# DanielaCourel/smoothed_particle_hydrodynamics

Measured on AMD Instinct MI355X. Metric: Mparticle-steps/sec (whole node), dam-break, higher is better.
Workload: dtype f32

## Files before the change

smoothed_particle_hydrodynamics_amd/csrc/full_tiled.h:

```cpp
#pragma once

#include "launch_policy.h"
#include "common_kernels.h"
#include "full_kernels.h"
#include "neighbor_lists.h"
#include "slab_kernels.h"

#if defined(SPH_ABLATE) && !defined(SPH_DIAGNOSTIC_BUILD)
#error "SPH_ABLATE is for diagnostic builds only: add -DSPH_DIAGNOSTIC_BUILD (tools/build_variant.sh does)"
#endif

#ifdef SPH_TRIPCOUNT
#ifndef SPH_DIAGNOSTIC_BUILD
#error "SPH_TRIPCOUNT is for diagnostic builds only: add -DSPH_DIAGNOSTIC_BUILD"
#endif
enum {
   TRIP_D_WAVES = 0, TRIP_D_CHUNKS_W, TRIP_D_TEST8_W, TRIP_D_TEST8_L, TRIP_D_SLOTS_L, TRIP_D_POPS_W,
   TRIP_D_POPS_L, TRIP_D_POPLOOPS_W, TRIP_D_SUMTRIPS_W, TRIP_D_SUMSLOTS_W, TRIP_D_LISTED_L, TRIP_D_LANES_L,
   TRIP_A_WAVES = 16, TRIP_A_PTRIPS_W, TRIP_A_CNT_L, TRIP_A_VTRIPS_W, TRIP_A_NV_L, TRIP_A_LANES_L,
   TRIP_COUNT = 32
};
__device__ unsigned long long g_trip[TRIP_COUNT];
struct TripCounters {
   unsigned int v[16];
// ... 703 lines not shown
   return block < count ? b1 + xcd_workgroup(block, count) : -1;
}

template <bool UNIT_SCALE>
__device__ __forceinline__ void fused_integrate(const FusedStep& fs, const PairConsts& k,
                                                const CellGrid& g, int p, bool live, float4 x,
                                                float4 a, int wg_index)
{
   double ke = 0.0, pe = 0.0;
   uint32_t c = 0xffffffffu;
   float4 v = make_float4(0.f, 0.f, 0.f, 0.f);
   if (live) {
      v = fs.velp_in[p];
      integrate_particle<UNIT_SCALE>(k, x, v, a, ke, pe);
      fs.posm_out[p] = x;
      fs.velp_out[p] = v;
      int cx, cy, cz;
      c = cell_of(g, x.x, x.y, x.z, cx, cy, cz);
      fs.key[p] = c;
   }
   count_cell_runs(c, live, p, fs.cell_count, fs.slot, (uint32_t)g.ncells);
   if (fs.slab) {
      bool to_left = false, to_right = false;
      if (live) {
         const int ob = fs.meta[META_OWN_BEGIN], oe = fs.meta[META_OWN_END];
         const int lo_end = min(fs.meta[META_BND_LO_END], oe);
         const int hi_begin = min(max(fs.meta[META_BND_HI_BEGIN], lo_end), oe);
         const int plane = cell_coord(x.z, g.inv, g.nz_global);
         const bool near_left = fs.zone.have_left && plane < fs.zone.lo + fs.zone.halo;
         const bool near_right = fs.zone.have_right && plane >= fs.zone.hi - fs.zone.halo;
         if ((p >= ob && p < lo_end) || (p >= hi_begin && p < oe)) {
            to_left = near_left;
            to_right = near_right;
         } else if (near_left || near_right) {
            atomicOr(&fs.meta[META_ERRORS], 8);
         }
      }
      if (fs.zone.have_left) {
         const int s = msg_reserve(&fs.left->header[0], to_left);
         if (to_left) {
            if (s < fs.msg_capacity) {
               fs.left->rec[2 * s] = x;
               fs.left->rec[2 * s + 1] = v;
            } else {
               atomicOr(&fs.meta[META_ERRORS], 2);
            }
         }
      }
      if (fs.zone.have_right) {
         const int s = msg_reserve(&fs.right->header[0], to_right);
         if (to_right) {
            if (s < fs.msg_capacity) {
               fs.right->rec[2 * s] = x;
               fs.right->rec[2 * s + 1] = v;
            } else {
               atomicOr(&fs.meta[META_ERRORS], 2);
            }
         }
      }
   }
   __shared__ double s_ke[TILE_THREADS / SPH_WAVE], s_pe[TILE_THREADS / SPH_WAVE];
#pragma unroll
   for (int d = SPH_WAVE / 2; d > 0; d >>= 1) {
      ke += __shfl_down(ke, d);
      pe += __shfl_down(pe, d);
   }
   const int lane = threadIdx.x & (SPH_WAVE - 1), w = threadIdx.x / SPH_WAVE;
   if (lane == 0) {
      s_ke[w] = ke;
      s_pe[w] = pe;
   }
   __syncthreads();
   if (threadIdx.x == 0) {
      double sa = 0.0, sb = 0.0;
#pragma unroll
      for (int q = 0; q < TILE_THREADS / SPH_WAVE; q++) {
         sa += s_ke[q];
         sb += s_pe[q];
      }
      fs.epart[2 * wg_index + 0] = sa;
      fs.epart[2 * wg_index + 1] = sb;
   }
   __syncthreads();
}

template <bool UNIT_SCALE, bool UNIFORM_MASS, bool WIDE, bool FAST>
__device__ __forceinline__ float4
accel_from_lists(int p, int cnt, const ListReader& lr, const TileDesc& d,
                 const float4* __restrict__ posm, const float4* __restrict__ velB,
                 const float* __restrict__ rho, const float* __restrict__ auxc, const PairConsts& k)
{
   const float4 pi = posm[p];
   AccelState s;
   accel_begin(k, s, pi, velB[p], rho[p]);
   const bool in_range = accel_operands_in_range(k);
   int first_v = 0;
   if (FAST) first_v = visc_first(cnt, s.visc_scale);
   if constexpr (FAST) {
      const int lastb = cnt > 0 ? (cnt - 1) >> 3 : 0;
      uint4 blk = lr.block(0);
      for (int j0 = 0; j0 < cnt; j0 += 8) {
         uint32_t entry[8];
         list_block_entries(blk, entry);
         blk = lr.block(min((j0 >> 3) + 1, lastb));
         float4 pj[8];
         float cj[8];
#pragma unroll
         for (int u = 0; u < 8; u++) {
            const uint32_t e = j0 + u < cnt ? entry[u] : entry[0];
            const int q = ListEntry<WIDE>::tile(e) - ListEntry<WIDE>::shift(d, e);
            pj[u] = posm[q];
            cj[u] = auxc[q];
         }
#pragma unroll
         for (int u = 0; u < 8; u++) {
            if (j0 + u < cnt) {
               float dx, dy, dz;
               float dd = sqrt_rn(dist2(pi.x, pi.y, pi.z, pj[u].x, pj[u].y, pj[u].z, dx, dy, dz));
               if (!UNIT_SCALE) dd *= k.sim_scale;
               accel_pair_fast_pressure<UNIT_SCALE>(k, s, dx, dy, dz, dd, cj[u]);
            }
         }
      }
      for (int j0 = first_v; j0 < cnt; j0 += VISC_UNROLL) {
         float4 pj[VISC_UNROLL], vj[VISC_UNROLL];
#pragma unroll
         for (int u = 0; u < VISC_UNROLL; u++) {
            const uint32_t e = lr.entry((uint32_t)min(j0 + u, cnt - 1));
            const int q = ListEntry<WIDE>::tile(e) - ListEntry<WIDE>::shift(d, e);
            pj[u] = posm[q];
            vj[u] = velB[q];
         }
#pragma unroll
         for (int u = 0; u < VISC_UNROLL; u++) {
            if (j0 + u < cnt) {
               float dx, dy, dz;
               float dd = sqrt_rn(dist2(pi.x, pi.y, pi.z, pj[u].x, pj[u].y, pj[u].z, dx, dy, dz));
               if (!UNIT_SCALE) dd *= k.sim_scale;
               accel_pair_fast_viscous(k, s, dd, vj[u].x, vj[u].y, vj[u].z, vj[u].w);
            }
         }
      }
      accel_fast_finish(k, s);
      return accel_end<UNIT_SCALE>(k, s);
   }
   constexpr int U = 4;
   for (int j0 = 0; j0 < cnt; j0 += U) {
      float4 pj[U], vj[U];
      float cj[U];
#pragma unroll
      for (int u = 0; u < U; u++) {
         const int j = min(j0 + u, cnt - 1);
         const uint32_t e = lr.entry((uint32_t)j);
         const int q = ListEntry<WIDE>::tile(e) - ListEntry<WIDE>::shift(d, e);
         pj[u] = posm[q];
         cj[u] = auxc[q];
         vj[u] = make_float4(0.f, 0.f, 0.f, 0.f);
         if (!FAST || j >= first_v) vj[u] = velB[q];
      }
#pragma unroll
      for (int u = 0; u < U; u++) {
         if (j0 + u < cnt) {
            float dx, dy, dz;
            const float d2 = dist2(pi.x, pi.y, pi.z, pj[u].x, pj[u].y, pj[u].z, dx, dy, dz);
            float dd = sqrt_rn(d2);
            if (!UNIT_SCALE) dd *= k.sim_scale;
            if (FAST) {
               accel_pair_fast_pressure<UNIT_SCALE>(k, s, dx, dy, dz, dd, cj[u]);
               if (j0 + u >= first_v) accel_pair_fast_viscous(k, s, dd, vj[u].x, vj[u].y, vj[u].z, vj[u].w);
            } else {
               accel_pair<UNIT_SCALE>(k, s, dx, dy, dz, dd, UNIFORM_MASS ? pi.w : pj[u].w, vj[u].x, vj[u].y,
                                      vj[u].z, vj[u].w, cj[u], in_range);
            }
         }
      }
   }
   if (FAST) accel_fast_finish(k, s);
   return accel_end<UNIT_SCALE>(k, s);
}

template <bool UNIT_SCALE, bool UNIFORM_MASS, bool WIDE, bool FAST>
__global__ void __launch_bounds__(TILE_THREADS, ACCEL_BLOCKS)
k_full_accel_lists(const float4* __restrict__ posm, const float4* __restrict__ velB,
                   const float* __restrict__ rho, const float* __restrict__ auxc,
                   const int32_t* __restrict__ ncount, const uint32_t* __restrict__ cell_start,
                   const int32_t* __restrict__ meta, CellGrid g, PairConsts k,
                   float4* __restrict__ acc, const TileDesc* __restrict__ desc,
                   const uint32_t* __restrict__ nlist, const uint32_t* __restrict__ nlist_overflow,
                   int tile_cap, const int32_t* __restrict__ tile_stats,
                   const uint32_t* __restrict__ giveup, int part, int list_cap,
                   int* __restrict__ tile_feedback, FusedStep fs, int tile_cap_density)
{
   PHASE_BEGIN();
   __shared__ AccelLds L;
   float4* xyzc = reinterpret_cast<float4*>(tile_lds_dynamic);
   constexpr int BATCH = TILE_BATCH;

   const int begin = meta[META_SUM_BEGIN], end = meta[META_SUM_END];
   const int ob = meta[META_OWN_BEGIN], oe = meta[META_OWN_END];
   const int tid = threadIdx.x;
   const int wgs = tile_stats[TSTAT_BLOCKS];
   const int mapped = accel_part_workgroup(part, blockIdx.x, wgs, begin, meta);
   const int wg = mapped < 0 ? 0 : mapped;
   const int p0 = begin + wg * TILE_THREADS;
   if (blockIdx.x == 0 && tid == 0) {
      tile_feedback[TSTAT_NO_LIST] = tile_stats[TSTAT_NO_LIST];
      if (fs.slab && part == 1) {
         if (fs.left) fs.left->header[1] = fs.msg_capacity;
         if (fs.right) fs.right->header[1] = fs.msg_capacity;
      }
   }
   const bool own = mapped >= 0 && !(p0 >= end || p0 + TILE_THREADS <= ob || p0 >= oe) &&
                    accel_part_has(part, p0, meta);
   const uint32_t gave_up = own ? nlist_overflow[wg] : LISTS_NONE;
   int desc_word = 0;
   if (tid < (int)(sizeof(TileDesc) / sizeof(int))) desc_word = reinterpret_cast<const int*>(&desc[wg])[tid];
   if ((int)blockIdx.x < tile_stats[TSTAT_GIVEUP_ACCEL]) {
      const int g0 = begin + (int)giveup[blockIdx.x] * TILE_THREADS;
      const int gp = g0 + tid;
      const bool mine = gp < end && gp >= ob && gp < oe && accel_part_has(part, g0, meta);
      const int gwg = (int)giveup[blockIdx.x];
      const uint32_t glists = nlist_overflow[gwg];
      if (glists != LISTS_NONE) {
         tile_desc_load(desc, gwg, L.desc);
         if (mine) {
            const int gcnt = ncount[gp];
            const ListReader glr(nlist, gwg, list_cap, tid);
            if (glists == LISTS_SOME && gcnt > 0 && glr.no_list())
               accel_untiled<UNIT_SCALE, FAST>(gp, posm, velB, rho, auxc, cell_start, g, k, acc, ncount);
            else
               acc[gp] = accel_from_lists<UNIT_SCALE, UNIFORM_MASS, WIDE, FAST>(gp, gcnt, glr, L.desc, posm, velB,
                                                                                rho, auxc, k);
         }
         __syncthreads();
      } else if (mine) {
         accel_untiled<UNIT_SCALE, FAST>(gp, posm, velB, rho, auxc, cell_start, g, k, acc, ncount);
      }
      if (fs.on && accel_part_has(part, g0, meta)) {
         float4 gx = make_float4(0.f, 0.f, 0.f, 0.f), ga = gx;
         if (mine) {
            gx = posm[gp];
            ga = acc[gp];
         }
         fused_integrate<UNIT_SCALE>(fs, k, g, gp, mine, gx, ga, (int)giveup[blockIdx.x]);
      }
   }
   if (gave_up == LISTS_NONE) return;
   if (tid < (int)(sizeof(TileDesc) / sizeof(int))) reinterpret_cast<int*>(&L.desc)[tid] = desc_word;
   __syncthreads();
   PHASE_MARK(16);
   const int total = L.desc.total;
   if (total > tile_cap || total > tile_cap_density) return;
   int B[9], D[9];
#pragma unroll
   for (int kk = 0; kk < 9; kk++) {
      B[kk] = L.desc.B[kk];
      D[kk] = L.desc.D[kk];
   }
   float4 buf[BATCH];
   float cbuf[BATCH];
#if defined(SPH_ABLATE) && SPH_ABLATE == 23
#pragma unroll
   for (int r = 0; r < BATCH; r++) {
      buf[r] = make_float4(0.f, 0.f, 0.f, 0.f);
      cbuf[r] = 0.f;
   }
   const int filled = 0;
#else
#pragma unroll
   for (int r = 0; r < BATCH; r++) {
      const int idx = min(tid + r * TILE_THREADS, total - 1);
      int d = D[0];
#pragma unroll
      for (int kk = 1; kk < 9; kk++) d = (idx >= B[kk]) ? D[kk] : d;
      buf[r] = posm[idx - d];
      cbuf[r] = auxc[idx - d];
   }
   const int filled = total;
#endif

   const int col = tid;
   const int p = p0 + col;
   const bool live = p < end && p >= ob && p < oe;
   float4 pi = make_float4(0.f, 0.f, 0.f, 0.f);
   float4 vi = pi;
   float rho_i = 0.0f;
   int cnt = 0;
   if (live) {
      pi = posm[p];
      vi = velB[p];
      rho_i = rho[p];
      cnt = ncount[p];
   }

   const ListReader lr(nlist, wg, list_cap, col);
   uint32_t entry[LIST_BLOCK_ENTRIES];
   uint4 next_blk = lr.block(0);

#pragma unroll
   for (int r = 0; r < BATCH; r++) {
      const int idx = tid + r * TILE_THREADS;
      if (idx < filled) xyzc[idx] = make_float4(buf[r].x, buf[r].y, buf[r].z, cbuf[r]);
   }
   for (int base = BATCH * TILE_THREADS; base < filled; base += BATCH * TILE_THREADS) {
#pragma unroll
      for (int r = 0; r < BATCH; r++) {
         const int idx = min(base + tid + r * TILE_THREADS, filled - 1);
         int d = D[0];
#pragma unroll
         for (int kk = 1; kk < 9; kk++) d = (idx >= B[kk]) ? D[kk] : d;
         buf[r] = posm[idx - d];
         cbuf[r] = auxc[idx - d];
      }
#pragma unroll
      for (int r = 0; r < BATCH; r++) {
         const int idx = base + tid + r * TILE_THREADS;
         if (idx < filled) xyzc[idx] = make_float4(buf[r].x, buf[r].y, buf[r].z, cbuf[r]);
      }
   }
   __syncthreads();

   PHASE_MARK(17);
   AccelState s;
   accel_begin(k, s, pi, vi, rho_i);
   const bool in_range = accel_operands_in_range(k);
   bool no_list = false;
   if (gave_up == LISTS_SOME && cnt > 0) no_list = next_blk.x == NLIST_NO_LIST;
   int first_v = 0;
   if (FAST) first_v = visc_first(cnt, s.visc_scale);
   if (no_list) cnt = 0;
#if defined(SPH_ABLATE) && (SPH_ABLATE == 21 || SPH_ABLATE == 23)
   cnt = 0;
#endif
   const int lastb = cnt > 0 ? (cnt - 1) >> 3 : 0;
   if constexpr (FAST) {
      const int self_tile = live ? p + L.desc.D[4] : 0;
      const float4 self = xyzc[self_tile];
      const float self_c = (k.hscaled * k.hscaled) * (s.pi_div_rhoi2 * self.w) +
                           ((self.x - self.x) + (self.y - self.y) + (self.z - self.z));
      const bool odd_lane = __any(!__builtin_isfinite(s.pi_div_rhoi2) || !__builtin_isfinite(self_c));
      TRIP(TripCounters trips; trips.wave(TRIP_A_WAVES - 16, true); trips.lane(TRIP_A_CNT_L - 16, (unsigned)cnt);
           trips.lane(TRIP_A_LANES_L - 16, live ? 1u : 0u); trips.lane(TRIP_A_NV_L - 16, (unsigned)(cnt - first_v));)
      for (int j0 = 0; __any(j0 < cnt); j0 += LIST_BLOCK_ENTRIES) {
         TRIP(trips.wave(TRIP_A_PTRIPS_W - 16, true);)
         list_block_entries(next_blk, entry);
         next_blk = lr.block(min((j0 >> 3) + 1, lastb));
         float dx[LIST_BLOCK_ENTRIES], dy[LIST_BLOCK_ENTRIES], dz[LIST_BLOCK_ENTRIES], dd[LIST_BLOCK_ENTRIES], bm[LIST_BLOCK_ENTRIES];
#pragma unroll
         for (int u = 0; u < LIST_BLOCK_ENTRIES; u++) {
            const bool valid = j0 + u < cnt;
            const float4 pj = xyzc[valid ? ListEntry<WIDE>::tile(entry[u]) : self_tile];
            dd[u] = dist2(pi.x, pi.y, pi.z, pj.x, pj.y, pj.z, dx[u], dy[u], dz[u]);
            bm[u] = pj.w;
         }
#if defined(SPH_ABLATE) && SPH_ABLATE == 22
#pragma unroll
         for (int u = 0; u < LIST_BLOCK_ENTRIES; u++) s.pgx += dd[u] + bm[u];
#else
         sqrt_rn_batch(dd);
         if (!odd_lane) {
#pragma unroll
            for (int u = 0; u < LIST_BLOCK_ENTRIES; u++) {
               if (!UNIT_SCALE) dd[u] *= k.sim_scale;
               accel_pair_fast_pressure<UNIT_SCALE>(k, s, dx[u], dy[u], dz[u], dd[u], bm[u]);
            }
         } else {
#pragma unroll
            for (int u = 0; u < LIST_BLOCK_ENTRIES; u++) {
               if (!UNIT_SCALE) dd[u] *= k.sim_scale;
               if (j0 + u < cnt) accel_pair_fast_pressure<UNIT_SCALE>(k, s, dx[u], dy[u], dz[u], dd[u], bm[u]);
            }
         }
#endif
      }
      PHASE_MARK(18);
      const int nv = cnt - first_v;
      TRIP(for (int m0 = 0; __any(m0 < nv); m0 += VISC_UNROLL) trips.wave(TRIP_A_VTRIPS_W - 16, true);
           trips.flush(16, 1u << (TRIP_A_CNT_L - 16) | 1u << (TRIP_A_NV_L - 16) | 1u << (TRIP_A_LANES_L - 16));)
      for (int m0 = 0; __any(m0 < nv); m0 += VISC_UNROLL) {
         float4 vj[VISC_UNROLL];
         int tj[VISC_UNROLL];
#pragma unroll
         for (int u = 0; u < VISC_UNROLL; u++) {
            const int j = min(first_v + m0 + u, cnt > 0 ? cnt - 1 : 0);
            const uint32_t e = lr.entry((uint32_t)j);
            tj[u] = ListEntry<WIDE>::tile(e);
            vj[u] = make_float4(0.f, 0.f, 0.f, 0.f);
            if (m0 + u < nv) vj[u] = velB[tj[u] - ListEntry<WIDE>::shift(L.desc, e)];
         }
#pragma unroll
         for (int u = 0; u < VISC_UNROLL; u++) {
            if (m0 + u < nv) {
               const float4 pj = xyzc[tj[u]];
               float dx, dy, dz;
               float d = sqrt_rn(dist2(pi.x, pi.y, pi.z, pj.x, pj.y, pj.z, dx, dy, dz));
               if (!UNIT_SCALE) d *= k.sim_scale;
               accel_pair_fast_viscous(k, s, d, vj[u].x, vj[u].y, vj[u].z, vj[u].w);
            }
         }
      }
   } else {
   for (int j0 = 0; __any(j0 < cnt); j0 += LIST_BLOCK_ENTRIES) {
      float4 vj[LIST_BLOCK_ENTRIES];
      float mj[LIST_BLOCK_ENTRIES];
      list_block_entries(next_blk, entry);
#pragma unroll
      for (int u = 0; u < LIST_BLOCK_ENTRIES; u++) {
         mj[u] = pi.w;
         const int q = ListEntry<WIDE>::tile(entry[u]) - ListEntry<WIDE>::shift(L.desc, entry[u]);
         const int qq = cnt > 0 ? q : p0;
#if defined(SPH_ABLATE) && SPH_ABLATE == 7
         vj[u] = make_float4(1.f, 2.f, 3.f, 4.f);
#else
         vj[u] = velB[qq];
#endif
         if (!UNIFORM_MASS) mj[u] = posm[qq].w;
      }
      next_blk = lr.block(min((j0 >> 3) + 1, lastb));
#pragma unroll
      for (int u = 0; u < LIST_BLOCK_ENTRIES; u++) {
         if (j0 + u < cnt) {
            const float4 pj = xyzc[ListEntry<WIDE>::tile(entry[u])];
            float dx, dy, dz;
            const float d2 = dist2(pi.x, pi.y, pi.z, pj.x, pj.y, pj.z, dx, dy, dz);
            float d = sqrt_rn(d2);
            if (!UNIT_SCALE) d *= k.sim_scale;
#if defined(SPH_ABLATE) && SPH_ABLATE == 22
            s.pgx += d + vj[u].x + pj.w;
#else
            accel_pair<UNIT_SCALE>(k, s, dx, dy, dz, d, mj[u], vj[u].x, vj[u].y, vj[u].z, vj[u].w,
                                   pj.w, in_range);
#endif
         }
      }
   }
   }
   if (gave_up == LISTS_SOME && __any(no_list) && no_list) {
      RowRanges rr;
      int cx, cy, cz;
      cell_of(g, pi.x, pi.y, pi.z, cx, cy, cz);
      row_ranges(g, cell_start, cx, cy, cz, rr);
      const int self_t = p + L.desc.D[4];
      int jw = 0;
#pragma unroll
      for (int kk = 0; kk < 9; kk++) {
         const int D = L.desc.D[kk];
         const int te = (int)rr.e[kk] + D;
         for (int t = (int)rr.s[kk] + D; t < te; t++) {
            const float4 pj = xyzc[t];
            float dx, dy, dz;
            const float d2 = dist2(pi.x, pi.y, pi.z, pj.x, pj.y, pj.z, dx, dy, dz);
            if (d2 < k.h2 && !(kk == 4 && t == self_t)) {
               float d = sqrt_rn(d2);
               if (!UNIT_SCALE) d *= k.sim_scale;
               if (FAST) {
                  accel_pair_fast_pressure<UNIT_SCALE>(k, s, dx, dy, dz, d, pj.w);
                  if (jw >= first_v) {
                     const float4 vj = velB[t - D];
                     accel_pair_fast_viscous(k, s, d, vj.x, vj.y, vj.z, vj.w);
                  }
                  jw++;
               } else {
                  const float4 vj = velB[t - D];
                  float mj = pi.w;
                  if (!UNIFORM_MASS) mj = posm[t - D].w;
                  accel_pair<UNIT_SCALE>(k, s, dx, dy, dz, d, mj, vj.x, vj.y, vj.z, vj.w, pj.w, in_range);
               }
            }
         }
      }
   }
   PHASE_MARK(19);
   if (FAST) accel_fast_finish(k, s);
   const float4 a_i = accel_end<UNIT_SCALE>(k, s);
   if (live) acc[p] = a_i;
   PHASE_MARK(20);
   if (fs.on) fused_integrate<UNIT_SCALE>(fs, k, g, p, live, pi, a_i, wg);
   PHASE_MARK(21);
   PHASE_COUNT(31);
}
```

smoothed_particle_hydrodynamics_amd/csrc/neighbor_lists.h:

```cpp
#pragma once

#include "launch_policy.h"
#include "sph_device.h"

constexpr int NLIST_CAP = 254;
#define NLIST_CAP_MAX 1022
#define LIST_BLOCK_ENTRIES 8
#define LIST_BLOCK_BYTES (16 * TILE_THREADS)
static_assert(NLIST_CAP <= NLIST_CAP_MAX, "initial list capacity");

__host__ __device__ __forceinline__ constexpr int list_rows(int list_cap)
{
   return 4 * ((list_cap + LIST_BLOCK_ENTRIES) / LIST_BLOCK_ENTRIES);
}

constexpr uint32_t LISTS_ALL = 0u;
constexpr uint32_t LISTS_NONE = 1u;
constexpr uint32_t LISTS_SOME = 2u;
#define NLIST_NO_LIST 0xffffffffu

__device__ __forceinline__ uint32_t list_entry_off(uint32_t j, uint32_t lane_off)
{
   return (j >> 3) * (uint32_t)LIST_BLOCK_BYTES + lane_off + (j & 7u) * 2u;
}
#define LIST_LANE_FIELD ((uint32_t)(LIST_BLOCK_BYTES - 16))
#define LIST_SLOT_FIELD 14u
__device__ __forceinline__ uint32_t list_pos_of(uint32_t j)
{
   return ((j >> 3) * (uint32_t)LIST_BLOCK_BYTES + (j & 7u) * 2u) | LIST_LANE_FIELD;
}
__device__ __forceinline__ uint32_t list_pos_off(uint32_t pos, uint32_t lane_off)
{
   return (LIST_LANE_FIELD & lane_off) | (~LIST_LANE_FIELD & pos);
}
__device__ __forceinline__ uint32_t list_pos_next(uint32_t pos) { return (pos + 2u) | LIST_LANE_FIELD; }
__device__ __forceinline__ uint32_t list_entry_load(const char* __restrict__ lists, uint32_t j, uint32_t lane_off)
{
   return *reinterpret_cast<const uint16_t*>(lists + list_entry_off(j, lane_off));
}
__device__ __forceinline__ uint4 list_block_load(const char* __restrict__ lists, int b, uint32_t lane_off)
{
   return *reinterpret_cast<const uint4*>(lists + (uint32_t)b * (uint32_t)LIST_BLOCK_BYTES + lane_off);
}
__device__ __forceinline__ void list_block_entries(const uint4& blk, uint32_t (&entry)[8])
{
   entry[0] = blk.x & 0xffffu; entry[1] = blk.x >> 16;
   entry[2] = blk.y & 0xffffu; entry[3] = blk.y >> 16;
   entry[4] = blk.z & 0xffffu; entry[5] = blk.z >> 16;
   entry[6] = blk.w & 0xffffu; entry[7] = blk.w >> 16;
}
__device__ __forceinline__ void list_pad(char* __restrict__ lists, uint32_t lane_off, int count, int list_cap)
{
   if (count >= list_cap + 1) return;
   uint32_t c = (uint32_t)count;
   if (c & 1u) { *reinterpret_cast<uint16_t*>(lists + list_entry_off(c, lane_off)) = (uint16_t)0; c += 1u; }
   if (c & 2u) { *reinterpret_cast<uint32_t*>(lists + list_entry_off(c, lane_off)) = 0u; c += 2u; }
   if (c & 4u) { *reinterpret_cast<uint2*>(lists + list_entry_off(c, lane_off)) = make_uint2(0u, 0u); }
}

template <bool WIDE>
struct ListEntry {
   static constexpr int TBITS = WIDE ? 14 : 12;
   static constexpr uint32_t TMASK = (1u << TBITS) - 1u;
   __device__ static __forceinline__ uint32_t tag(int segment)
   {
      return (uint32_t)(WIDE ? segment / 3 : segment) << TBITS;
   }
   __device__ static __forceinline__ int tile(uint32_t e) { return (int)(e & TMASK); }
   template <class Desc>
   __device__ static __forceinline__ int shift(const Desc& d, uint32_t e)
   {
      if (!WIDE) return d.D[e >> TBITS];
      const int z = (int)(e >> TBITS), t = (int)(e & TMASK);
      const int k = 3 * z + (t >= d.B[3 * z + 1] ? 1 : 0) + (t >= d.B[3 * z + 2] ? 1 : 0);
      return d.D[k];
   }
};
static_assert(TILE_CAP_MAX + TILE_PAD <= (1 << ListEntry<false>::TBITS) &&
                 TILE_CAP_MAX_WIDE + TILE_PAD <= (1 << ListEntry<true>::TBITS),
              "tile index must fit the list entry");

template <class Word>
__device__ __forceinline__ Word* list_block_of(Word* nlist, int wg, int list_cap)
{
   return nlist + (size_t)wg * (size_t)(list_rows(list_cap) * TILE_THREADS);
}

struct ListReader {
   const char* lists;
   uint32_t lane_off;
   __device__ __forceinline__ ListReader(const uint32_t* nlist, int wg, int list_cap, int lane)
      : lists(reinterpret_cast<const char*>(list_block_of(nlist, wg, list_cap))), lane_off(16u * (uint32_t)lane)
   {
   }
   __device__ __forceinline__ uint4 block(int b) const { return list_block_load(lists, b, lane_off); }
   __device__ __forceinline__ uint32_t entry(uint32_t j) const { return list_entry_load(lists, j, lane_off); }
   __device__ __forceinline__ bool no_list() const
   {
      return *reinterpret_cast<const uint32_t*>(lists + lane_off) == NLIST_NO_LIST;
   }
};

__device__ __forceinline__ void list_stage_clear(char* stage_lane)
{
   *reinterpret_cast<uint4*>(stage_lane) = make_uint4(0u, 0u, 0u, 0u);
}

struct ListWriter {
   char* lists;
   uint32_t lane_off;
   char* stage;
   __device__ __forceinline__ ListWriter(uint32_t* nlist, int wg, int list_cap, int lane, char* stage_lane)
      : lists(reinterpret_cast<char*>(list_block_of(nlist, wg, list_cap))), lane_off(16u * (uint32_t)lane),
        stage(stage_lane)
   {
   }
   template <bool STAGED>
   __device__ __forceinline__ void append(uint32_t& pos, uint32_t e)
   {
      const uint32_t in_block = pos & LIST_SLOT_FIELD;
      if constexpr (STAGED) {
         *reinterpret_cast<uint16_t*>(stage + in_block) = (uint16_t)e;
         if (in_block == LIST_SLOT_FIELD)
            *reinterpret_cast<uint4*>(lists + list_pos_off(pos & ~LIST_SLOT_FIELD, lane_off)) =
               *reinterpret_cast<const uint4*>(stage);
      } else {
         *reinterpret_cast<uint16_t*>(lists + list_pos_off(pos, lane_off)) = (uint16_t)e;
      }
      pos = list_pos_next(pos);
   }
   __device__ __forceinline__ uint4 block(int b) const { return list_block_load(lists, b, lane_off); }
   __device__ __forceinline__ void keep(int kept, uint32_t e)
   {
      *reinterpret_cast<uint16_t*>(lists + list_entry_off((uint32_t)kept, lane_off)) = (uint16_t)e;
   }
   __device__ __forceinline__ void pad(int count, int list_cap) { list_pad(lists, lane_off, count, list_cap); }
   __device__ __forceinline__ bool finish(uint32_t pos, int count, int list_cap, bool staged, int& wg_no_list)
   {
      if (!staged)
         list_pad(lists, lane_off, count, list_cap);
      else if (count <= list_cap && ((count & 7) != 0 || count == 0))
         *reinterpret_cast<uint4*>(lists + list_pos_off(pos & ~LIST_SLOT_FIELD, lane_off)) =
            *reinterpret_cast<const uint4*>(stage);
      const bool none = count > list_cap;
      if (none) {
         wg_no_list = 1;
         *reinterpret_cast<uint32_t*>(lists + lane_off) = NLIST_NO_LIST;
      }
      return none;
   }
};

__device__ __forceinline__ void lists_publish(bool no_list, const int& wg_no_list, int32_t* tile_stats,
                                              uint32_t* nlist_overflow, int wg)
{
   if (__any(no_list)) {
      const int without = __popcll(__ballot(no_list));
      if ((threadIdx.x & (SPH_WAVE - 1)) == 0) atomicAdd(&tile_stats[TSTAT_NO_LIST], without);
   }
   __syncthreads();
   if (threadIdx.x == 0) nlist_overflow[wg] = wg_no_list ? LISTS_SOME : LISTS_ALL;
}
```

Measured before the change: 4685.

## Prefetch first viscous neighbor velocities during tile staging and run viscous pass first

In the fast path, the state setup and the first four viscous-pass list entries are computed before the tile-staging loop. Their velocities are loaded from global memory while the staging loads are still in flight, so that latency overlaps the barrier. The viscous loop now runs before the pressure loop and starts from the prefetched batch. The cost is more live registers across the staging loop, which may hurt occupancy. Reordering the loops also changes the floating-point accumulation order if the two passes share accumulators.

```diff
diff --git a/smoothed_particle_hydrodynamics_amd/csrc/full_tiled.h b/smoothed_particle_hydrodynamics_amd/csrc/full_tiled.h
--- a/smoothed_particle_hydrodynamics_amd/csrc/full_tiled.h
+++ b/smoothed_particle_hydrodynamics_amd/csrc/full_tiled.h
@@ -1029,6 +1029,27 @@
       const int idx = tid + r * TILE_THREADS;
       if (idx < filled) xyzc[idx] = make_float4(buf[r].x, buf[r].y, buf[r].z, cbuf[r]);
    }
+
+   AccelState s;
+   int first_v = 0;
+   bool no_list = false;
+   float4 vpre[VISC_UNROLL];
+   int tpre[VISC_UNROLL], nvp = 0;
+   uint32_t ev[VISC_UNROLL];
+   if constexpr (FAST) {
+      static_assert(VISC_UNROLL == 4, "list_entries_from takes four entries");
+      accel_begin(k, s, pi, vi, rho_i);
+      first_v = visc_first(cnt, s.visc_scale);
+      const int lcnt = cnt <= list_cap ? cnt : 0;
+      const int fv = lcnt > 0 ? first_v : 0;
+      const int lb = lcnt > 0 ? (lcnt - 1) >> 3 : 0;
+      const int fb = fv >> 3;
+      const uint4 blk_a = lr.block(fb), blk_b = lr.block(min(fb + 1, lb));
+      if (gave_up == LISTS_SOME && cnt > 0) no_list = next_blk.x == NLIST_NO_LIST;
+      nvp = no_list ? 0 : lcnt - fv;
+      list_entries_from(blk_a, blk_b, (uint32_t)(fv & 7), ev);
+   }
+
    for (int base = BATCH * TILE_THREADS; base < filled; base += BATCH * TILE_THREADS) {
 #pragma unroll
       for (int r = 0; r < BATCH; r++) {
@@ -1045,66 +1066,44 @@
          if (idx < filled) xyzc[idx] = make_float4(buf[r].x, buf[r].y, buf[r].z, cbuf[r]);
       }
    }
+   if constexpr (FAST) {
+#pragma unroll
+      for (int u = 0; u < VISC_UNROLL; u++) {
+         tpre[u] = ListEntry<WIDE>::tile(ev[u]);
+         vpre[u] = make_float4(0.f, 0.f, 0.f, 0.f);
+         if (u < nvp) vpre[u] = velB[tpre[u] - ListEntry<WIDE>::shift(L.desc, ev[u])];
+      }
+   }
    __syncthreads();
 
    PHASE_MARK(17);
-   AccelState s;
-   accel_begin(k, s, pi, vi, rho_i);
+   if constexpr (!FAST) accel_begin(k, s, pi, vi, rho_i);
    const bool in_range = accel_operands_in_range(k);
-   bool no_list = false;
-   if (gave_up == LISTS_SOME && cnt > 0) no_list = next_blk.x == NLIST_NO_LIST;
-   int first_v = 0;
-   if (FAST) first_v = visc_first(cnt, s.visc_scale);
+   if constexpr (!FAST) {
+      if (gave_up == LISTS_SOME && cnt > 0) no_list = next_blk.x == NLIST_NO_LIST;
+   }
    if (no_list) cnt = 0;
 #if defined(SPH_ABLATE) && (SPH_ABLATE == 21 || SPH_ABLATE == 23)
    cnt = 0;
 #endif
    const int lastb = cnt > 0 ? (cnt - 1) >> 3 : 0;
    if constexpr (FAST) {
-      const int self_tile = live ? p + L.desc.D[4] : 0;
-      const float4 self = xyzc[self_tile];
-      const float self_c = (k.hscaled * k.hscaled) * (s.pi_div_rhoi2 * self.w) +
-                           ((self.x - self.x) + (self.y - self.y) + (self.z - self.z));
-      const bool odd_lane = __any(!__builtin_isfinite(s.pi_div_rhoi2) || !__builtin_isfinite(self_c));
       TRIP(TripCounters trips; trips.wave(TRIP_A_WAVES - 16, true); trips.lane(TRIP_A_CNT_L - 16, (unsigned)cnt);
            trips.lane(TRIP_A_LANES_L - 16, live ? 1u : 0u); trips.lane(TRIP_A_NV_L - 16, (unsigned)(cnt - first_v));)
-      for (int j0 = 0; __any(j0 < cnt); j0 += LIST_BLOCK_ENTRIES) {
-         TRIP(trips.wave(TRIP_A_PTRIPS_W - 16, true);)
-         list_block_entries(next_blk, entry);
-         next_blk = lr.block(min((j0 >> 3) + 1, lastb));
-         float dx[LIST_BLOCK_ENTRIES], dy[LIST_BLOCK_ENTRIES], dz[LIST_BLOCK_ENTRIES], dd[LIST_BLOCK_ENTRIES], bm[LIST_BLOCK_ENTRIES];
-#pragma unroll
-         for (int u = 0; u < LIST_BLOCK_ENTRIES; u++) {
-            const bool valid = j0 + u < cnt;
-            const float4 pj = xyzc[valid ? ListEntry<WIDE>::tile(entry[u]) : self_tile];
-            dd[u] = dist2(pi.x, pi.y, pi.z, pj.x, pj.y, pj.z, dx[u], dy[u], dz[u]);
-            bm[u] = pj.w;
-         }
-#if defined(SPH_ABLATE) && SPH_ABLATE == 22
-#pragma unroll
-         for (int u = 0; u < LIST_BLOCK_ENTRIES; u++) s.pgx += dd[u] + bm[u];
-#else
-         sqrt_rn_batch(dd);
-         if (!odd_lane) {
-#pragma unroll
-            for (int u = 0; u < LIST_BLOCK_ENTRIES; u++) {
-               if (!UNIT_SCALE) dd[u] *= k.sim_scale;
-               accel_pair_fast_pressure<UNIT_SCALE>(k, s, dx[u], dy[u], dz[u], dd[u], bm[u]);
-            }
-         } else {
-#pragma unroll
-            for (int u = 0; u < LIST_BLOCK_ENTRIES; u++) {
-               if (!UNIT_SCALE) dd[u] *= k.sim_scale;
-               if (j0 + u < cnt) accel_pair_fast_pressure<UNIT_SCALE>(k, s, dx[u], dy[u], dz[u], dd[u], bm[u]);
-            }
-         }
-#endif
-      }
-      PHASE_MARK(18);
       const int nv = cnt - first_v;
-      TRIP(for (int m0 = 0; __any(m0 < nv); m0 += VISC_UNROLL) trips.wave(TRIP_A_VTRIPS_W - 16, true);
-           trips.flush(16, 1u << (TRIP_A_CNT_L - 16) | 1u << (TRIP_A_NV_L - 16) | 1u << (TRIP_A_LANES_L - 16));)
-      for (int m0 = 0; __any(m0 < nv); m0 += VISC_UNROLL) {
+      if (__any(0 < nv)) {
+#pragma unroll
+         for (int u = 0; u < VISC_UNROLL; u++) {
+            if (u < nv) {
+               const float4 pj = xyzc[tpre[u]];
+               float dx, dy, dz;
+               float d = sqrt_rn(dist2(pi.x, pi.y, pi.z, pj.x, pj.y, pj.z, dx, dy, dz));
+               if (!UNIT_SCALE) d *= k.sim_scale;
+               accel_pair_fast_viscous(k, s, d, vpre[u].x, vpre[u].y, vpre[u].z, vpre[u].w);
+            }
+         }
+      }
+      for (int m0 = VISC_UNROLL; __any(m0 < nv); m0 += VISC_UNROLL) {
          float4 vj[VISC_UNROLL];
          int tj[VISC_UNROLL];
 #pragma unroll
@@ -1126,6 +1125,46 @@
             }
          }
       }
+      PHASE_MARK(18);
+      const int self_tile = live ? p + L.desc.D[4] : 0;
+      const float4 self = xyzc[self_tile];
+      const float self_c = (k.hscaled * k.hscaled) * (s.pi_div_rhoi2 * self.w) +
+                           ((self.x - self.x) + (self.y - self.y) + (self.z - self.z));
+      const bool odd_lane = __any(!__builtin_isfinite(s.pi_div_rhoi2) || !__builtin_isfinite(self_c));
+      for (int j0 = 0; __any(j0 < cnt); j0 += LIST_BLOCK_ENTRIES) {
+         TRIP(trips.wave(TRIP_A_PTRIPS_W - 16, true);)
+         list_block_entries(next_blk, entry);
+         next_blk = lr.block(min((j0 >> 3) + 1, lastb));
+         float dx[LIST_BLOCK_ENTRIES], dy[LIST_BLOCK_ENTRIES], dz[LIST_BLOCK_ENTRIES], dd[LIST_BLOCK_ENTRIES], bm[LIST_BLOCK_ENTRIES];
+#pragma unroll
+         for (int u = 0; u < LIST_BLOCK_ENTRIES; u++) {
+            const bool valid = j0 + u < cnt;
+            const float4 pj = xyzc[valid ? ListEntry<WIDE>::tile(entry[u]) : self_tile];
+            dd[u] = dist2(pi.x, pi.y, pi.z, pj.x, pj.y, pj.z, dx[u], dy[u], dz[u]);
+            bm[u] = pj.w;
+         }
+#if defined(SPH_ABLATE) && SPH_ABLATE == 22
+#pragma unroll
+         for (int u = 0; u < LIST_BLOCK_ENTRIES; u++) s.pgx += dd[u] + bm[u];
+#else
+         sqrt_rn_batch(dd);
+         if (!odd_lane) {
+#pragma unroll
+            for (int u = 0; u < LIST_BLOCK_ENTRIES; u++) {
+               if (!UNIT_SCALE) dd[u] *= k.sim_scale;
+               accel_pair_fast_pressure<UNIT_SCALE>(k, s, dx[u], dy[u], dz[u], dd[u], bm[u]);
+            }
+         } else {
+#pragma unroll
+            for (int u = 0; u < LIST_BLOCK_ENTRIES; u++) {
+               if (!UNIT_SCALE) dd[u] *= k.sim_scale;
+               if (j0 + u < cnt) accel_pair_fast_pressure<UNIT_SCALE>(k, s, dx[u], dy[u], dz[u], dd[u], bm[u]);
+            }
+         }
+#endif
+      }
+      TRIP(for (int m0 = 0; __any(m0 < nv); m0 += VISC_UNROLL) trips.wave(TRIP_A_VTRIPS_W - 16, true);
+           trips.flush(16, 1u << (TRIP_A_CNT_L - 16) | 1u << (TRIP_A_NV_L - 16) | 1u << (TRIP_A_LANES_L - 16));)
    } else {
    for (int j0 = 0; __any(j0 < cnt); j0 += LIST_BLOCK_ENTRIES) {
       float4 vj[LIST_BLOCK_ENTRIES];
diff --git a/smoothed_particle_hydrodynamics_amd/csrc/neighbor_lists.h b/smoothed_particle_hydrodynamics_amd/csrc/neighbor_lists.h
--- a/smoothed_particle_hydrodynamics_amd/csrc/neighbor_lists.h
+++ b/smoothed_particle_hydrodynamics_amd/csrc/neighbor_lists.h
@@ -48,6 +48,18 @@
    entry[2] = blk.y & 0xffffu; entry[3] = blk.y >> 16;
    entry[4] = blk.z & 0xffffu; entry[5] = blk.z >> 16;
    entry[6] = blk.w & 0xffffu; entry[7] = blk.w >> 16;
+}
+__device__ __forceinline__ void list_entries_from(const uint4& a, const uint4& b, uint32_t first, uint32_t (&entry)[4])
+{
+   const uint32_t w = first >> 1;
+   const uint32_t w0 = w == 0u ? a.x : w == 1u ? a.y : w == 2u ? a.z : a.w;
+   const uint32_t w1 = w == 0u ? a.y : w == 1u ? a.z : w == 2u ? a.w : b.x;
+   const uint32_t w2 = w == 0u ? a.z : w == 1u ? a.w : w == 2u ? b.x : b.y;
+   const uint32_t sh = (first & 1u) * 16u;
+   const uint32_t lo = (uint32_t)((((uint64_t)w1 << 32) | w0) >> sh);
+   const uint32_t hi = (uint32_t)((((uint64_t)w2 << 32) | w1) >> sh);
+   entry[0] = lo & 0xffffu; entry[1] = lo >> 16;
+   entry[2] = hi & 0xffffu; entry[3] = hi >> 16;
 }
 __device__ __forceinline__ void list_pad(char* __restrict__ lists, uint32_t lane_off, int count, int list_cap)
 {
```

Measured after the change: 4761, median of 6. +1.6%, better.
